# Borda/pyImSegm

Hardware: NVIDIA H100
Metric: megapixels/sec end-to-end SLIC+features+GC (pipe_color2d_slic_features_model_graphcut) (higher is better)
Workload: dtype f64

## Files before the change

include/imsegm_b200.h:

```cpp
#ifndef IMSEGM_B200_H
#define IMSEGM_B200_H

#include <stddef.h>
#include <stdint.h>

#ifdef __cplusplus
extern "C" {
#endif

typedef void* isb_stream_t;

enum isb_status {
    ISB_OK = 0,
    ISB_ERR_ARG = -1,
    ISB_ERR_CUDA = -2,
    ISB_ERR_CAPACITY = -3,
    ISB_ERR_UNSUPPORTED = -4
};

enum isb_dtype { ISB_U8 = 0, ISB_U16 = 1, ISB_F32 = 2, ISB_F64 = 3 };

const char* isb_last_error(void);
int isb_abi_version(void);
long long isb_launch_count(void);
// ... 2 lines not shown
int isb_profile_stage_count(void);
const char* isb_profile_stage_name(int id);
int isb_profile_collect(double* ms_out , long long* count_out );


int isb_slic_prepare(const void* img, int dtype, int H, int W, int C, const double* w_half, int radius, double ratio,
                     int rescale, double* lab_planar, double* minmax_out , isb_stream_t stream);

int isb_image_minmax(const void* img, int dtype, long long n, double* minmax_out , isb_stream_t stream);

size_t isb_slic_kmeans_workspace_bytes(int H, int W, int n_seeds, int step_y, int step_x);

int isb_slic_kmeans(const double* lab_planar, int H, int W, const double* seeds_yx, int n_seeds, int step_y, int step_x,
                    double step, int max_iter, int slic_zero, int32_t* labels, double* centroids, void* ws, size_t ws_bytes,
                    isb_stream_t stream);

typedef struct isb_slic_band {
    int32_t slab_rows, width;
    int32_t image_rows, y_off;
    int32_t own_lo, own_hi;
    int32_t halo;
    int32_t n_seeds, step_y, step_x, slic_zero;
    double step;
    const double* lab_slab;
    size_t plane_stride;
    const double* seeds_yx;
    int32_t* labels_slab;
    void* ws; size_t ws_bytes;
} isb_slic_band_t;
int isb_slic_band_begin(const isb_slic_band_t* band, isb_stream_t stream);
// ... 161 lines not shown
```

pyimsegm_b200/_lib.py:

```python
import ctypes as C
import os

_HERE = os.path.dirname(os.path.abspath(__file__))
LIB_PATH = os.path.join(_HERE, 'libimsegm_b200.so')

_lib = None

ISB_OK, ISB_ERR_ARG, ISB_ERR_CUDA, ISB_ERR_CAPACITY, ISB_ERR_UNSUPPORTED = 0, -1, -2, -3, -4
DTYPE_CODES = {'uint8': 0, 'uint16': 1, 'float32': 2, 'float64': 3}

_vp, _i, _d, _sz, _ll = C.c_void_p, C.c_int, C.c_double, C.c_size_t, C.c_longlong



class SlicBand(C.Structure):
    _fields_ = [('slab_rows', C.c_int32), ('width', C.c_int32), ('image_rows', C.c_int32), ('y_off', C.c_int32),
                ('own_lo', C.c_int32), ('own_hi', C.c_int32), ('halo', C.c_int32),
                ('n_seeds', C.c_int32), ('step_y', C.c_int32), ('step_x', C.c_int32), ('slic_zero', C.c_int32),
                ('step', C.c_double), ('lab_slab', C.c_void_p), ('plane_stride', C.c_size_t), ('seeds_yx', C.c_void_p),
                ('labels_slab', C.c_void_p), ('ws', C.c_void_p), ('ws_bytes', C.c_size_t)]


_bp = C.POINTER(SlicBand)

# ... 6 lines not shown
    'isb_profile_stage_count': (_i, []),
    'isb_profile_stage_name': (C.c_char_p, [_i]),
    'isb_profile_collect': (_i, [C.POINTER(_d), C.POINTER(_ll)]),
    'isb_slic_prepare': (_i, [_vp, _i, _i, _i, _i, C.POINTER(_d), _i, _d, _i, _vp, _vp, _vp]),
    'isb_image_minmax': (_i, [_vp, _i, _ll, _vp, _vp]),
    'isb_slic_band_begin': (_i, [_bp, _vp]),
    'isb_slic_band_assign': (_i, [_bp, _vp]),
    'isb_slic_band_update': (_i, [_bp, _vp, _vp]),
    'isb_slic_band_import': (_i, [_bp, _vp, _vp, _vp]),
    'isb_slic_band_finalize': (_i, [_bp, _vp, _vp]),
    'isb_segment_stats_accumulate': (_i, [_vp, _i, _vp, _i, _i, _i, _i, _vp, _vp, _vp]),
    'isb_segment_stats_deviation': (_i, [_vp, _i, _vp, _i, _i, _i, _vp, _vp, _vp, _vp, _vp]),
    'isb_segment_stats_finish': (_i, [_i, _i, _vp, _vp, _vp, _vp, _i, _i, _vp, _vp, _vp]),
    'isb_slic_kmeans_workspace_bytes': (_sz, [_i, _i, _i, _i, _i]),
    'isb_slic_kmeans': (_i, [_vp, _i, _i, _vp, _i, _i, _i, _d, _i, _i, _vp, _vp, _vp, _sz, _vp]),
    'isb_slic3d_prepare': (_i, [_vp, _i, _i, _i, _i, _vp, _i, _vp, _i, _vp, _i, _d, _vp, _vp, _vp]),
    'isb_slic3d_kmeans_workspace_bytes': (_sz, [_i, _i, _i, _i]),
    'isb_slic3d_kmeans': (_i, [_vp, _i, _i, _i, _vp, _i, _i, _i, _i, _d, C.POINTER(_d), _i, _vp, _vp, _sz, _vp]),
    'isb_connectivity3d_workspace_bytes': (_sz, [_i, _i, _i, _i]),
    'isb_enforce_connectivity3d': (_i, [_vp, _i, _i, _i, _i, _i, _vp, _vp, _vp, _sz, _vp]),
    'isb_connectivity_workspace_bytes': (_sz, [_i, _i]),
    'isb_enforce_connectivity': (_i, [_vp, _i, _i, _i, _i, _vp, _vp, _vp, _sz, _vp]),
    'isb_segment_stats_workspace_bytes': (_sz, [_i]),
    'isb_segment_stats_2d': (_i, [_vp, _i, _vp, _i, _i, _i, _i, _vp, _i, _i, _vp, _vp, _vp, _sz, _vp]),
    'isb_adjacency_workspace_bytes': (_sz, [_i, _i]),
    'isb_adjacency_edges': (_i, [_vp, _i, _i, _i, _vp, _i, _vp, _vp, _sz, _vp]),
    'isb_adjacency_edges_3d': (_i, [_vp, _i, _i, _i, _i, _vp, _i, _vp, _vp, _sz, _vp]),
    'isb_centroids_3d': (_i, [_vp, _i, _i, _i, _i, _vp, _vp, _sz, _vp]),
    'isb_gc_energies_workspace_bytes': (_sz, [_i, _i, _i]),
    'isb_gc_energies': (_i, [_vp, _i, _vp, _i, _vp, _i, _vp, _vp, _i, _i, _d, _vp, _vp, _vp, _vp, _vp, _vp, _vp, _sz, _vp]),
# ... 99 lines not shown
```

pyimsegm_b200/csrc/slic_kmeans.cu:

```cuda
#include "common.cuh"
#include "wgmma.cuh"
#include <float.h>
#include <string.h>

namespace {

constexpr int TILE = 32;
constexpr int ACAP = 128;
constexpr int AROWS = 8;
constexpr int AWARPS = TILE / AROWS;
constexpr int ATHREADS = 32 * AWARPS;


struct __align__(16) Cand {
    double cy, cx, c0, c1, c2;
    int y0, y1, x0, x1;
    int k, pad;
};
static_assert(sizeof(Cand) == 64, "Cand must be 64 bytes");

struct KmState {
    double* cy; double* cx; double* c0; double* c1; double* c2;
    int4* win;
    int4* obb;
    int* bin_start;
    int* bin_fill;
    int* bin_of;
    int* pack_done;
    Cand* packed;
    double* packed_maxdc;
    unsigned long long* maxdc;
    int slico;
    int n, H, W, step_y, step_x, B, nby, nbx;
    double sw;
    int Hg, y_off, own_lo, own_hi, halo;
    size_t pstride;
};

__device__ __forceinline__ int4 make_window(double cy, double cx, int step_y, int step_x, int H, int W)
{
    double lo, hi;
    int4 w;
    lo = __dsub_rn(cy, (double)(2 * step_y)); if (0.0 > lo) lo = 0.0;
    hi = __dadd_rn(__dadd_rn(cy, (double)(2 * step_y)), 1.0); if ((double)H < hi) hi = (double)H;
    w.x = (int)lo; w.y = (int)hi;
    lo = __dsub_rn(cx, (double)(2 * step_x)); if (0.0 > lo) lo = 0.0;
    hi = __dadd_rn(__dadd_rn(cx, (double)(2 * step_x)), 1.0); if ((double)W < hi) hi = (double)W;
    w.z = (int)lo; w.w = (int)hi;
    return w;
}

__global__ void k_seed(KmState s, const double* __restrict__ seeds_yx)
{
    const int k = blockIdx.x * blockDim.x + threadIdx.x;
    if (k >= s.n) return;
    const double cy = seeds_yx[2 * k], cx = seeds_yx[2 * k + 1];
    s.cy[k] = cy; s.cx[k] = cx; s.c0[k] = 0.0; s.c1[k] = 0.0; s.c2[k] = 0.0;
    s.win[k] = make_window(cy, cx, s.step_y, s.step_x, s.Hg, s.W);
    const int by = min(max((int)cy / s.B, 0), s.nby - 1), bx = min(max((int)cx / s.B, 0), s.nbx - 1);
    s.bin_of[k] = by * s.nbx + bx;
    atomicAdd(&s.bin_fill[by * s.nbx + bx], 1);
    s.obb[k] = make_int4(INT_MAX, -1, INT_MAX, -1);
    s.maxdc[k] = (unsigned long long)__double_as_longlong(1.0);
}

__global__ void __launch_bounds__(1024) k_scan_bins(KmState s)
{
    const int nbins = s.nby * s.nbx;
    __shared__ int s_wsum[32];
    __shared__ int s_part_total;
    __shared__ int s_carry;
    if (threadIdx.x == 0) { s_carry = 0; *s.pack_done = 0; }
    __syncthreads();
    const int lane = threadIdx.x & 31, wid = threadIdx.x >> 5, nw = blockDim.x >> 5;
    for (int base = 0; base < nbins; base += blockDim.x) {
        int b = base + threadIdx.x;
        int v = b < nbins ? s.bin_fill[b] : 0;
        int incl = v;
#pragma unroll
        for (int o = 1; o < 32; o <<= 1) { int t = __shfl_up_sync(0xffffffffu, incl, o); if (lane >= o) incl += t; }
        if (lane == 31) s_wsum[wid] = incl;
        __syncthreads();
        if (wid == 0) {
            int t = lane < nw ? s_wsum[lane] : 0, ti = t;
#pragma unroll
            for (int o = 1; o < 32; o <<= 1) { int u = __shfl_up_sync(0xffffffffu, ti, o); if (lane >= o) ti += u; }
            s_wsum[lane] = ti - t;
            if (lane == 31) s_part_total = ti;
        }
        __syncthreads();
        const int carry = s_carry;
        if (b < nbins) { s.bin_start[b] = carry + s_wsum[wid] + incl - v; s.bin_fill[b] = 0; }
        __syncthreads();
        if (threadIdx.x == 0) s_carry = carry + s_part_total;
        __syncthreads();
    }
    if (threadIdx.x == 0) s.bin_start[nbins] = s_carry;
}

__global__ void __launch_bounds__(256) k_pack(KmState s)
{
    const int k = blockIdx.x * blockDim.x + threadIdx.x;
    if (k < s.n) {
        const int bin = s.bin_of[k];
        if (bin >= 0) {
            const int pos = s.bin_start[bin] + atomicAdd(&s.bin_fill[bin], 1);
            const int4 w = s.win[k];
            Cand c;
            c.cy = s.cy[k]; c.cx = s.cx[k]; c.c0 = s.c0[k]; c.c1 = s.c1[k]; c.c2 = s.c2[k];
            c.y0 = w.x; c.y1 = w.y; c.x0 = w.z; c.x1 = w.w; c.k = k; c.pad = 0;
            s.packed[pos] = c;
            if (s.slico) s.packed_maxdc[pos] = __longlong_as_double((long long)s.maxdc[k]);
        }
    }
    __shared__ int s_last;
    __syncthreads();
    if (threadIdx.x == 0) { __threadfence(); s_last = atomicAdd(s.pack_done, 1) == (int)gridDim.x - 1; }
    __syncthreads();
    if (s_last) {
        const int nbins = s.nby * s.nbx;
        for (int b = threadIdx.x; b < nbins; b += blockDim.x) s.bin_fill[b] = 0;
    }
}

__device__ __forceinline__ unsigned long long dbits(double v) { return (unsigned long long)__double_as_longlong(v); }

template <bool SLICO>
__global__ void __launch_bounds__(ATHREADS, 5) k_assign(const __grid_constant__ CUtensorMap lab_map, int use_tma, KmState s,
                                                        const double* __restrict__ lab, int* __restrict__ labels)
{
    __shared__ Cand cand[ACAP];
    __shared__ double s_maxdc[SLICO ? ACAP : 1];
    __shared__ float s_key[ACAP];
    __shared__ float2 s_cf[ACAP];
    __shared__ double s_lb[ACAP];
    __shared__ unsigned char s_order[ACAP];
    __shared__ __align__(128) double s_px[3][TILE][TILE];
    __shared__ __align__(8) unsigned long long s_bar;
    __shared__ int s_ncand, s_done, s_row, s_off, s_total;
    const int tx0 = blockIdx.x * TILE, ty0 = blockIdx.y * TILE;
    const int tx1 = min(tx0 + TILE, s.W);
    const int gy0 = ty0 + s.y_off, gy1 = min(ty0 + TILE, s.H) + s.y_off;
    const int lane = threadIdx.x & 31, warp = threadIdx.x >> 5;
    const size_t HW = s.pstride;
    const int x = tx0 + lane;
    const bool xin = x < s.W;
    const int yb = ty0 + warp * AROWS;

    double best[AROWS];
    int bestk[AROWS];
#pragma unroll
    for (int j = 0; j < AROWS; ++j) { best[j] = DBL_MAX; bestk[j] = -1; }
    if (use_tma) {
        if (threadIdx.x == 0) {
            wgmma::mbar_init(wgmma::smem_u32(&s_bar), 1);
            wgmma::fence_mbar_init();
            wgmma::mbar_arrive_expect_tx(wgmma::smem_u32(&s_bar), 3 * TILE * TILE * 8);
            wgmma::tma_load_3d(wgmma::smem_u32(&s_px[0][0][0]), &lab_map, tx0, ty0, 0, wgmma::smem_u32(&s_bar));
        }
    } else {
        double v[3][AROWS];
#pragma unroll
        for (int j = 0; j < AROWS; ++j) {
            const int y = yb + j;
            if (xin && y < s.H) {
                const size_t p = (size_t)y * s.W + x;
                v[0][j] = lab[p]; v[1][j] = lab[HW + p]; v[2][j] = lab[2 * HW + p];
            } else { v[0][j] = v[1][j] = v[2][j] = 0.0; }
        }
#pragma unroll
        for (int j = 0; j < AROWS; ++j) {
            s_px[0][warp * AROWS + j][lane] = v[0][j]; s_px[1][warp * AROWS + j][lane] = v[1][j]; s_px[2][warp * AROWS + j][lane] = v[2][j];
        }
    }
    const int by0 = max(gy0 - 2 * s.step_y - 2, 0) / s.B, by1 = min(gy1 + 2 * s.step_y + 1, s.Hg - 1) / s.B;
    const int bx0 = max(tx0 - 2 * s.step_x - 2, 0) / s.B, bx1 = min(tx1 + 2 * s.step_x + 1, s.W - 1) / s.B;
    const float tcy = 0.5f * (gy0 + gy1 - 1), tcx = 0.5f * (tx0 + tx1 - 1);
    const int byl = min(by1, s.nby - 1), bxl = min(bx1, s.nbx - 1);
    if (threadIdx.x == 0) { s_row = by0; s_off = 0; s_done = 0; s_ncand = 0; s_total = 0; }
    __syncthreads();
    if (warp == 0) {
        int t = 0;
        for (int row = by0 + lane; row <= byl; row += 32) t += s.bin_start[row * s.nbx + bxl + 1] - s.bin_start[row * s.nbx + bx0];
#pragma unroll
        for (int o = 16; o > 0; o >>= 1) t += __shfl_xor_sync(0xffffffffu, t, o);
        if (lane == 0) s_total = t;
    }
    __syncthreads();
    const bool fast = s_total <= ACAP;

    while (true) {
        if (fast) {
            for (int row = by0 + warp; row <= byl; row += AWARPS) {
                const int beg = s.bin_start[row * s.nbx + bx0], end = s.bin_start[row * s.nbx + bxl + 1];
                for (int i = beg + lane; i < end; i += 32) {
                    const Cand c = s.packed[i];
                    if ((c.y0 < gy1) && (c.y1 > gy0) && (c.x0 < tx1) && (c.x1 > tx0)) {
                        const int pos = atomicAdd(&s_ncand, 1);
                        cand[pos] = c;
                        if (SLICO) s_maxdc[pos] = s.packed_maxdc[i];
                        const float fy = (float)c.cy - tcy, fx = (float)c.cx - tcx;
                        s_key[pos] = fy * fy + fx * fx;
                        s_cf[pos] = make_float2((float)c.cy, (float)c.cx);
                    }
                }
            }
            if (threadIdx.x == 0) s_done = 1;
        } else if (warp == 0) {
            int n = 0;
            int row = s_row, off = s_off;
            while (row <= byl && n < ACAP) {
                int beg = s.bin_start[row * s.nbx + bx0] + off;
                int end = s.bin_start[row * s.nbx + bxl + 1];
                while (beg < end && n < ACAP) {
                    int room = ACAP - n;
                    int i = beg + lane;
                    bool ok = false;
                    Cand c;
                    if (i < end && lane < room) {
                        c = s.packed[i];
                        ok = (c.y0 < gy1) && (c.y1 > gy0) && (c.x0 < tx1) && (c.x1 > tx0);
                    }
                    unsigned m = __ballot_sync(0xffffffffu, ok);
                    if (ok) {
                        int pos = n + __popc(m & ((1u << lane) - 1u));
                        cand[pos] = c;
                        if (SLICO) s_maxdc[pos] = s.packed_maxdc[i];
                        const float fy = (float)c.cy - tcy, fx = (float)c.cx - tcx;
                        s_key[pos] = fy * fy + fx * fx;
                        s_cf[pos] = make_float2((float)c.cy, (float)c.cx);
                    }
                    n += __popc(m);
                    int adv = min(min(32, room), end - beg);
                    beg += adv; off += adv;
                }
                if (beg >= end) { ++row; off = 0; }
            }
            if (lane == 0) { s_ncand = n; s_row = row; s_off = off; s_done = row > byl; }
        }
        __syncthreads();
        const int nc = s_ncand;
        const int done = s_done;
        for (int t = threadIdx.x; t < nc; t += ATHREADS) {
            const float key = s_key[t];
            int rank = 0;
            for (int j = 0; j < nc; ++j) {
                const float kj = s_key[j];
                rank += (kj < key) || (kj == key && j < t);
            }
            s_order[rank] = (unsigned char)t;
            const float r = sqrtf(key) - 23.5f;
            s_lb[rank] = r > 0.f ? (double)(r * r * 0.999f) * s.sw * 0.999 : 0.0;
        }
        __syncthreads();
        if (use_tma) wgmma::mbar_wait(wgmma::smem_u32(&s_bar), 0);
        if (xin) {
            const double xd = (double)x;
            const float xf = (float)x, ymid = (float)(yb + s.y_off) + 0.5f * (AROWS - 1), swf = (float)s.sw * 0.998f;
            unsigned long long worst = dbits(DBL_MAX);
#pragma unroll
            for (int j = 0; j < AROWS; ++j) worst = max(worst, dbits(best[j]));
            float worstf = __double2float_ru(__longlong_as_double((long long)worst));
            for (int ci = 0; ci < nc; ++ci) {
                if (dbits(s_lb[ci]) > worst) break;
                const int c = s_order[ci];
                {
                    const float2 cf = s_cf[c];
                    const float ax = fmaxf(fabsf(cf.y - xf) - 2e-3f, 0.f), ay = fmaxf(fabsf(cf.x - ymid) - (0.5f * (AROWS - 1) + 2e-3f), 0.f);
                    if ((ax * ax + ay * ay) * swf > worstf) continue;
                }
                const int cx0 = cand[c].x0, cx1 = cand[c].x1;
                if (x < cx0 || x >= cx1) continue;
                const int cy0 = cand[c].y0, ck = cand[c].k;
                const unsigned cyn = (unsigned)(cand[c].y1 - cy0);
                const double ccy = cand[c].cy;
                const double tx = __dsub_rn(cand[c].cx, xd);
                const double dx2 = __dmul_rn(tx, tx);
                bool improved = false;
#pragma unroll
                for (int jg = 0; jg < AROWS; jg += 4) {
                    double sp[4];
                    bool need[4];
#pragma unroll
                    for (int q = 0; q < 4; ++q) {
// ... 71 lines not shown
    if (b) asm volatile("bar.arrive %0, %1;" ::"n"(ID + 1), "n"(N) : "memory");
    else asm volatile("bar.arrive %0, %1;" ::"n"(ID), "n"(N) : "memory");
}

template <bool BAND>
__global__ void __launch_bounds__(UTHREADS, UBLOCKS) k_update(KmState s, const double* __restrict__ lab, const int* __restrict__ labels,
                                                              long long* __restrict__ xchg)
{
    __shared__ __align__(16) double buf[2][3][USTRIDE];
    __shared__ int s_cnt[2][USTRIP];
    __shared__ int s_tot[2];
    __shared__ long long s_int[UGATHER][3];
    __shared__ double s_acc[3];
    __shared__ int4 s_box;
    __shared__ int s_skip;
    const int lane = threadIdx.x & 31, wl = threadIdx.x >> 5;
    const int k = s.n - 1 - blockIdx.x;
    if (threadIdx.x == 0) {
        const int4 o = s.obb[k];
        int skip = 0;
        if (BAND) {
            const bool alive = s.bin_of[k] >= 0;
            const int cr = alive ? (int)s.cy[k] : 0;
            if (o.y >= o.x && (!alive || o.x + s.y_off < cr - s.halo || o.y + s.y_off > cr + s.halo))
                atomicAdd((unsigned long long*)&xchg[6 * (size_t)s.n], 1ull);
            s.obb[k] = make_int4(INT_MAX, -1, INT_MAX, -1);
            skip = !alive || cr < s.own_lo || cr >= s.own_hi;
        }
        s_box = o; s_skip = skip;
    }
    __syncthreads();
    if (s_skip) return;
    const int4 o = s_box;
    const int y0 = o.x, y1 = o.y + 1, x0 = o.z, x1 = o.w + 1;
    const int nchunk = (x1 > x0) ? (x1 - x0 + 31) / 32 : 0;
    const int total = (y1 > y0) ? (y1 - y0) * nchunk : 0;
    const int nstrip = (total + USTRIP - 1) / USTRIP;
// ... 72 lines not shown
                const double2* bsrc = reinterpret_cast<const double2*>(buf[b][lane]);
                const int ng = (s_tot[b] + 3) >> 2;
                double2 c01 = bsrc[0], c23 = bsrc[1];
                for (int g = 1; g <= ng; ++g) {
                    const double2 n01 = bsrc[2 * g], n23 = bsrc[2 * g + 1];
                    acc = __dadd_rn(__dadd_rn(__dadd_rn(__dadd_rn(acc, c01.x), c01.y), c23.x), c23.y);
                    c01 = n01; c23 = n23;
                }
            }
            __syncwarp();
            if (i + 2 < nstrip) bar_arrive<UBAR_EMPTY, UTHREADS>(b);
        }
        if (lane < 3) s_acc[lane] = acc;
    }
    __syncthreads();
    if (threadIdx.x != 0) return;
    long long cnt = 0, sy = 0, sx = 0;
#pragma unroll
    for (int w = 0; w < UGATHER; ++w) { cnt += s_int[w][0]; sy += s_int[w][1]; sx += s_int[w][2]; }
    const double a0 = s_acc[0], a1 = s_acc[1], a2 = s_acc[2];
    if (BAND) {
        long long* r = xchg + 6 * (size_t)k;
        if (cnt > 0) {
            const double dn = (double)cnt;
            r[0] = __double_as_longlong(__ddiv_rn((double)sy, dn)); r[1] = __double_as_longlong(__ddiv_rn((double)sx, dn));
            r[2] = __double_as_longlong(__ddiv_rn(a0, dn)); r[3] = __double_as_longlong(__ddiv_rn(a1, dn));
            r[4] = __double_as_longlong(__ddiv_rn(a2, dn));
            r[5] = 1;
        } else r[5] = 2;
        return;
    }
    int4 w = make_int4(0, 0, 0, 0);
    int bin = -1;
    if (cnt > 0) {
        const double dn = (double)cnt;
        const double cy = __ddiv_rn((double)sy, dn), cx = __ddiv_rn((double)sx, dn);
        s.cy[k] = cy; s.cx[k] = cx;
        s.c0[k] = __ddiv_rn(a0, dn); s.c1[k] = __ddiv_rn(a1, dn); s.c2[k] = __ddiv_rn(a2, dn);
        w = make_window(cy, cx, s.step_y, s.step_x, s.Hg, s.W);
        const int by = min(max((int)cy / s.B, 0), s.nby - 1), bx = min(max((int)cx / s.B, 0), s.nbx - 1);
        bin = by * s.nbx + bx;
        atomicAdd(&s.bin_fill[bin], 1);
    }
    s.win[k] = w;
    s.bin_of[k] = bin;
    s.obb[k] = make_int4(INT_MAX, -1, INT_MAX, -1);
}

__global__ void k_import(KmState s, const long long* __restrict__ xchg)
{
    const int k = blockIdx.x * blockDim.x + threadIdx.x;
    if (k >= s.n) return;
    const long long* r = xchg + 6 * (size_t)k;
    const long long state = r[5];
    if (state == 1) {
        const double cy = __longlong_as_double(r[0]), cx = __longlong_as_double(r[1]);
        s.cy[k] = cy; s.cx[k] = cx;
        s.c0[k] = __longlong_as_double(r[2]); s.c1[k] = __longlong_as_double(r[3]); s.c2[k] = __longlong_as_double(r[4]);
        s.win[k] = make_window(cy, cx, s.step_y, s.step_x, s.Hg, s.W);
        const int by = min(max((int)cy / s.B, 0), s.nby - 1), bx = min(max((int)cx / s.B, 0), s.nbx - 1);
        s.bin_of[k] = by * s.nbx + bx;
        atomicAdd(&s.bin_fill[by * s.nbx + bx], 1);
    } else {
        s.win[k] = make_int4(0, 0, 0, 0);
        s.bin_of[k] = -1;
    }
}

__global__ void __launch_bounds__(256) k_slico_max(KmState s, const double* __restrict__ lab, const int* __restrict__ labels)
{
    const size_t HW = s.pstride;
    const size_t first = (size_t)(s.own_lo - s.y_off) * s.W, npx = (size_t)(s.own_hi - s.own_lo) * s.W;
    const size_t q = (size_t)blockIdx.x * blockDim.x + threadIdx.x;
    if (q >= npx) return;
    const size_t p = first + q;
    const int k = labels[p];
    const double d0 = __dsub_rn(lab[p], s.c0[k]), d1 = __dsub_rn(lab[HW + p], s.c1[k]), d2 = __dsub_rn(lab[2 * HW + p], s.c2[k]);
    double dcol = __dmul_rn(d0, d0);
    dcol = __dadd_rn(dcol, __dmul_rn(d1, d1));
    dcol = __dadd_rn(dcol, __dmul_rn(d2, d2));
    if (dcol == dcol) atomicMax(&s.maxdc[k], (unsigned long long)__double_as_longlong(dcol));
}

__global__ void k_export_centroids(KmState s, double* out)
{
    int k = blockIdx.x * blockDim.x + threadIdx.x;
    if (k >= s.n) return;
    out[5 * k] = s.cy[k]; out[5 * k + 1] = s.cx[k];
    out[5 * k + 2] = s.c0[k]; out[5 * k + 3] = s.c1[k]; out[5 * k + 4] = s.c2[k];
}

static size_t carve(KmState& s, void* ws, size_t bytes, int H, int W, int n, int step_y, int step_x)
{
    WsCarver c(ws, bytes);
    s.n = n; s.H = H; s.W = W; s.step_y = step_y; s.step_x = step_x;
    s.Hg = H; s.y_off = 0; s.own_lo = 0; s.own_hi = H; s.halo = 0; s.pstride = (size_t)H * W;
    s.B = 2 * (step_y > step_x ? step_y : step_x);
    if (s.B < 16) s.B = 16;
    s.nby = (H + s.B - 1) / s.B; s.nbx = (W + s.B - 1) / s.B;
    s.cy = c.take<double>(n); s.cx = c.take<double>(n);
    s.c0 = c.take<double>(n); s.c1 = c.take<double>(n); s.c2 = c.take<double>(n);
    s.win = c.take<int4>(n); s.obb = c.take<int4>(n);
    s.bin_start = c.take<int>((size_t)s.nby * s.nbx + 1);
    s.bin_fill = c.take<int>((size_t)s.nby * s.nbx);
    s.bin_of = c.take<int>(n);
    s.pack_done = c.take<int>(1);
    s.packed = c.take<Cand>(n);
    s.maxdc = c.take<unsigned long long>(n);
    s.packed_maxdc = c.take<double>(n);
    return isb_align(c.off);
}

static int rebin(KmState& s, const double* seeds_yx, cudaStream_t st)
{
    if (seeds_yx) {
        ISB_CUDA_CHECK(cudaMemsetAsync(s.bin_fill, 0, sizeof(int) * (size_t)s.nby * s.nbx, st));
        k_seed<<<(s.n + 255) / 256, 256, 0, st>>>(s, seeds_yx);
        ISB_LAUNCH_CHECK();
    }
    k_scan_bins<<<1, 1024, 0, st>>>(s);
    ISB_LAUNCH_CHECK();
    k_pack<<<(s.n + 255) / 256, 256, 0, st>>>(s);
    ISB_LAUNCH_CHECK();
    return ISB_OK;
}

static bool make_lab_map(CUtensorMap& map, const double* lab, int rows, int W, size_t plane_stride)
{
    wgmma::EncodeTiledFn encode = wgmma::encode_tiled_fn();
    if (!encode || (W & 1) || (plane_stride & 1) || ((uintptr_t)lab & 15)) return false;
    const cuuint64_t gdim[3] = { (cuuint64_t)W, (cuuint64_t)rows, 3 };
    const cuuint64_t gstride[2] = { (cuuint64_t)W * sizeof(double), (cuuint64_t)plane_stride * sizeof(double) };
    const cuuint32_t box[3] = { TILE, TILE, 3 };
    const cuuint32_t estr[3] = { 1, 1, 1 };
    return encode(&map, CU_TENSOR_MAP_DATA_TYPE_FLOAT64, 3, (void*)lab, gdim, gstride, box, estr, CU_TENSOR_MAP_INTERLEAVE_NONE,
                  CU_TENSOR_MAP_SWIZZLE_NONE, CU_TENSOR_MAP_L2_PROMOTION_L2_256B, CU_TENSOR_MAP_FLOAT_OOB_FILL_NONE) == CUDA_SUCCESS;
}
// ... 14 lines not shown
}

extern "C" int isb_slic_kmeans(const double* lab_planar, int H, int W, const double* seeds_yx, int n_seeds, int step_y,
                               int step_x, double step, int max_iter, int slic_zero, int32_t* labels, double* centroids,
                               void* ws, size_t ws_bytes, isb_stream_t stream)
{
    ISB_REQUIRE(lab_planar && seeds_yx && labels && ws, "null pointer");
    ISB_REQUIRE(H > 0 && W > 0 && n_seeds > 0 && step_y > 0 && step_x > 0 && step > 0, "bad sizes");
    KmState s;
    size_t need = carve(s, ws, ws_bytes, H, W, n_seeds, step_y, step_x);
    ISB_REQUIRE(need <= ws_bytes, "workspace too small");
    s.sw = 1.0 / (step * step);
    s.slico = slic_zero ? 1 : 0;
    cudaStream_t st = (cudaStream_t)stream;
    ISB_CUDA_CHECK(cudaMemsetAsync(labels, 0, sizeof(int32_t) * (size_t)H * W, st));
    if (int rc = rebin(s, seeds_yx, st)) return rc;
    CUtensorMap lab_map;
    memset(&lab_map, 0, sizeof(lab_map));
    const int use_tma = make_lab_map(lab_map, lab_planar, H, W, s.pstride) ? 1 : 0;
    for (int it = 0; it < max_iter; ++it) {
        {
            ProfScope p(ISB_PROF_ASSIGN, st);
            launch_assign(s, lab_map, use_tma, lab_planar, labels, st);
        }
        ISB_LAUNCH_CHECK();
        { ProfScope p(ISB_PROF_UPDATE, st); k_update<false><<<n_seeds, UTHREADS, 0, st>>>(s, lab_planar, labels, nullptr); }
        ISB_LAUNCH_CHECK();
        if (slic_zero) {
            const size_t npx = (size_t)H * W;
            k_slico_max<<<(unsigned)((npx + 255) / 256), 256, 0, st>>>(s, lab_planar, labels);
            ISB_LAUNCH_CHECK();
        }
        { ProfScope p(ISB_PROF_FINALIZE, st); if (int rc = rebin(s, nullptr, st)) return rc; }
    }
    if (centroids) {
        k_export_centroids<<<(n_seeds + 255) / 256, 256, 0, st>>>(s, centroids);
        ISB_LAUNCH_CHECK();
    }
    return ISB_OK;
}

namespace {

static int band_state(const isb_slic_band_t* b, KmState& s)
{
    ISB_REQUIRE(b && b->lab_slab && b->seeds_yx && b->labels_slab && b->ws, "null pointer");
    ISB_REQUIRE(b->slab_rows > 0 && b->width > 0 && b->image_rows > 0 && b->n_seeds > 0 && b->step_y > 0 && b->step_x > 0 && b->step > 0,
                "bad sizes");
// ... 9 lines not shown
    s.H = b->slab_rows; s.Hg = b->image_rows; s.y_off = b->y_off; s.own_lo = b->own_lo; s.own_hi = b->own_hi; s.halo = b->halo;
    s.pstride = b->plane_stride;
    s.sw = 1.0 / (b->step * b->step);
    s.slico = b->slic_zero ? 1 : 0;
    return ISB_OK;
}

}

extern "C" int isb_slic_band_begin(const isb_slic_band_t* b, isb_stream_t stream)
{
    KmState s;
    if (int rc = band_state(b, s)) return rc;
    cudaStream_t st = (cudaStream_t)stream;
    ISB_CUDA_CHECK(cudaMemsetAsync(b->labels_slab, 0, sizeof(int32_t) * (size_t)b->slab_rows * b->width, st));
    return rebin(s, b->seeds_yx, st);
}

extern "C" int isb_slic_band_assign(const isb_slic_band_t* b, isb_stream_t stream)
{
    KmState s;
    if (int rc = band_state(b, s)) return rc;
    cudaStream_t st = (cudaStream_t)stream;
    CUtensorMap lab_map;
    memset(&lab_map, 0, sizeof(lab_map));
    const int use_tma = make_lab_map(lab_map, b->lab_slab, s.H, s.W, s.pstride) ? 1 : 0;
    ProfScope p(ISB_PROF_ASSIGN, st);
    launch_assign(s, lab_map, use_tma, b->lab_slab, b->labels_slab, st);
    ISB_LAUNCH_CHECK();
    return ISB_OK;
}
// ... 25 lines not shown
        ISB_LAUNCH_CHECK();
        ISB_CUDA_CHECK(cudaMemcpyAsync(maxdc_xchg, s.maxdc, sizeof(uint64_t) * (size_t)s.n, cudaMemcpyDeviceToDevice, st));
    }
    return ISB_OK;
}

extern "C" int isb_slic_band_finalize(const isb_slic_band_t* b, const uint64_t* maxdc_xchg, isb_stream_t stream)
{
    KmState s;
    if (int rc = band_state(b, s)) return rc;
    cudaStream_t st = (cudaStream_t)stream;
    if (s.slico) {
        ISB_REQUIRE(maxdc_xchg, "null pointer");
        ISB_CUDA_CHECK(cudaMemcpyAsync(s.maxdc, maxdc_xchg, sizeof(uint64_t) * (size_t)s.n, cudaMemcpyDeviceToDevice, st));
    }
    ProfScope p(ISB_PROF_FINALIZE, st);
    return rebin(s, nullptr, st);
}
```

Before: 1381.

## Replace seed binning with per-tile candidate lists and add a color-bound prune

Drops the bin scan/pack pipeline (scan_bins and pack kernels run every iteration). The update kernel now appends each centroid straight into per-tile candidate lists via atomics, and the assign kernel reads its own tile's list directly, falling back to a full scan when a tile overflows its capacity. The assign loop also adds a color-space lower bound from per-warp pixel min/max in float with directed rounding, to skip distance evaluations. The cost is tile-list memory, atomic contention, and nondeterministic candidate order, plus a tile-cap knob and a full-scan counter for testing.

```diff
diff --git a/include/imsegm_b200.h b/include/imsegm_b200.h
--- a/include/imsegm_b200.h
+++ b/include/imsegm_b200.h
@@ -40,6 +40,9 @@
 int isb_slic_kmeans(const double* lab_planar, int H, int W, const double* seeds_yx, int n_seeds, int step_y, int step_x,
                     double step, int max_iter, int slic_zero, int32_t* labels, double* centroids, void* ws, size_t ws_bytes,
                     isb_stream_t stream);
+
+int isb_slic_set_tile_cap(int cap);
+long long isb_slic_full_scan_tiles(void);
 
 typedef struct isb_slic_band {
     int32_t slab_rows, width;
diff --git a/pyimsegm_b200/_lib.py b/pyimsegm_b200/_lib.py
--- a/pyimsegm_b200/_lib.py
+++ b/pyimsegm_b200/_lib.py
@@ -44,6 +44,8 @@
     'isb_segment_stats_finish': (_i, [_i, _i, _vp, _vp, _vp, _vp, _i, _i, _vp, _vp, _vp]),
     'isb_slic_kmeans_workspace_bytes': (_sz, [_i, _i, _i, _i, _i]),
     'isb_slic_kmeans': (_i, [_vp, _i, _i, _vp, _i, _i, _i, _d, _i, _i, _vp, _vp, _vp, _sz, _vp]),
+    'isb_slic_set_tile_cap': (_i, [_i]),
+    'isb_slic_full_scan_tiles': (_ll, []),
     'isb_slic3d_prepare': (_i, [_vp, _i, _i, _i, _i, _vp, _i, _vp, _i, _vp, _i, _d, _vp, _vp, _vp]),
     'isb_slic3d_kmeans_workspace_bytes': (_sz, [_i, _i, _i, _i]),
     'isb_slic3d_kmeans': (_i, [_vp, _i, _i, _i, _vp, _i, _i, _i, _i, _d, C.POINTER(_d), _i, _vp, _vp, _sz, _vp]),
diff --git a/pyimsegm_b200/csrc/slic_kmeans.cu b/pyimsegm_b200/csrc/slic_kmeans.cu
--- a/pyimsegm_b200/csrc/slic_kmeans.cu
+++ b/pyimsegm_b200/csrc/slic_kmeans.cu
@@ -23,15 +23,11 @@
     double* cy; double* cx; double* c0; double* c1; double* c2;
     int4* win;
     int4* obb;
-    int* bin_start;
-    int* bin_fill;
-    int* bin_of;
-    int* pack_done;
-    Cand* packed;
-    double* packed_maxdc;
+    int* tile_cnt;
+    Cand* tile_cand;
     unsigned long long* maxdc;
     int slico;
-    int n, H, W, step_y, step_x, B, nby, nbx;
+    int n, H, W, step_y, step_x, ntx, tcap;
     double sw;
     int Hg, y_off, own_lo, own_hi, halo;
     size_t pstride;
@@ -50,115 +46,93 @@
     return w;
 }
 
+__device__ __forceinline__ Cand make_cand(int k, double cy, double cx, double c0, double c1, double c2, int4 w)
+{
+    Cand c;
+    c.cy = cy; c.cx = cx; c.c0 = c0; c.c1 = c1; c.c2 = c2;
+    c.y0 = w.x; c.y1 = w.y; c.x0 = w.z; c.x1 = w.w; c.k = k; c.pad = 0;
+    return c;
+}
+
+__device__ __forceinline__ void append_tiles(const KmState& s, const Cand& c, int t, int nt)
+{
+    const int ya = max(c.y0 - s.y_off, 0), yb = min(c.y1 - s.y_off, s.H);
+    if (ya >= yb || c.x0 >= c.x1) return;
+    const int ty0 = ya / TILE, tx0 = c.x0 / TILE;
+    const int nx = (c.x1 - 1) / TILE - tx0 + 1, nxy = ((yb - 1) / TILE - ty0 + 1) * nx;
+    for (int i = t; i < nxy; i += nt) {
+        const int tile = (ty0 + i / nx) * s.ntx + tx0 + i % nx;
+        const int pos = atomicAdd(&s.tile_cnt[tile], 1);
+        if (pos < s.tcap) s.tile_cand[(size_t)tile * s.tcap + pos] = c;
+    }
+}
+
 __global__ void k_seed(KmState s, const double* __restrict__ seeds_yx)
 {
     const int k = blockIdx.x * blockDim.x + threadIdx.x;
     if (k >= s.n) return;
     const double cy = seeds_yx[2 * k], cx = seeds_yx[2 * k + 1];
     s.cy[k] = cy; s.cx[k] = cx; s.c0[k] = 0.0; s.c1[k] = 0.0; s.c2[k] = 0.0;
-    s.win[k] = make_window(cy, cx, s.step_y, s.step_x, s.Hg, s.W);
-    const int by = min(max((int)cy / s.B, 0), s.nby - 1), bx = min(max((int)cx / s.B, 0), s.nbx - 1);
-    s.bin_of[k] = by * s.nbx + bx;
-    atomicAdd(&s.bin_fill[by * s.nbx + bx], 1);
+    const int4 w = make_window(cy, cx, s.step_y, s.step_x, s.Hg, s.W);
+    s.win[k] = w;
     s.obb[k] = make_int4(INT_MAX, -1, INT_MAX, -1);
     s.maxdc[k] = (unsigned long long)__double_as_longlong(1.0);
-}
-
-__global__ void __launch_bounds__(1024) k_scan_bins(KmState s)
-{
-    const int nbins = s.nby * s.nbx;
-    __shared__ int s_wsum[32];
-    __shared__ int s_part_total;
-    __shared__ int s_carry;
-    if (threadIdx.x == 0) { s_carry = 0; *s.pack_done = 0; }
-    __syncthreads();
-    const int lane = threadIdx.x & 31, wid = threadIdx.x >> 5, nw = blockDim.x >> 5;
-    for (int base = 0; base < nbins; base += blockDim.x) {
-        int b = base + threadIdx.x;
-        int v = b < nbins ? s.bin_fill[b] : 0;
-        int incl = v;
-#pragma unroll
-        for (int o = 1; o < 32; o <<= 1) { int t = __shfl_up_sync(0xffffffffu, incl, o); if (lane >= o) incl += t; }
-        if (lane == 31) s_wsum[wid] = incl;
-        __syncthreads();
-        if (wid == 0) {
-            int t = lane < nw ? s_wsum[lane] : 0, ti = t;
-#pragma unroll
-            for (int o = 1; o < 32; o <<= 1) { int u = __shfl_up_sync(0xffffffffu, ti, o); if (lane >= o) ti += u; }
-            s_wsum[lane] = ti - t;
-            if (lane == 31) s_part_total = ti;
-        }
-        __syncthreads();
-        const int carry = s_carry;
-        if (b < nbins) { s.bin_start[b] = carry + s_wsum[wid] + incl - v; s.bin_fill[b] = 0; }
-        __syncthreads();
-        if (threadIdx.x == 0) s_carry = carry + s_part_total;
-        __syncthreads();
-    }
-    if (threadIdx.x == 0) s.bin_start[nbins] = s_carry;
-}
-
-__global__ void __launch_bounds__(256) k_pack(KmState s)
-{
-    const int k = blockIdx.x * blockDim.x + threadIdx.x;
-    if (k < s.n) {
-        const int bin = s.bin_of[k];
-        if (bin >= 0) {
-            const int pos = s.bin_start[bin] + atomicAdd(&s.bin_fill[bin], 1);
-            const int4 w = s.win[k];
-            Cand c;
-            c.cy = s.cy[k]; c.cx = s.cx[k]; c.c0 = s.c0[k]; c.c1 = s.c1[k]; c.c2 = s.c2[k];
-            c.y0 = w.x; c.y1 = w.y; c.x0 = w.z; c.x1 = w.w; c.k = k; c.pad = 0;
-            s.packed[pos] = c;
-            if (s.slico) s.packed_maxdc[pos] = __longlong_as_double((long long)s.maxdc[k]);
-        }
-    }
-    __shared__ int s_last;
-    __syncthreads();
-    if (threadIdx.x == 0) { __threadfence(); s_last = atomicAdd(s.pack_done, 1) == (int)gridDim.x - 1; }
-    __syncthreads();
-    if (s_last) {
-        const int nbins = s.nby * s.nbx;
-        for (int b = threadIdx.x; b < nbins; b += blockDim.x) s.bin_fill[b] = 0;
-    }
+    append_tiles(s, make_cand(k, cy, cx, 0.0, 0.0, 0.0, w), 0, 1);
 }
 
 __device__ __forceinline__ unsigned long long dbits(double v) { return (unsigned long long)__double_as_longlong(v); }
+
+__device__ unsigned long long d_full_scans;
+
+struct __align__(16) CandF {
+    float cy, cx, inv, pad0;
+    float lo0, lo1, lo2, pad1;
+    float hi0, hi1, hi2, pad2;
+};
 
 template <bool SLICO>
 __global__ void __launch_bounds__(ATHREADS, 5) k_assign(const __grid_constant__ CUtensorMap lab_map, int use_tma, KmState s,
                                                         const double* __restrict__ lab, int* __restrict__ labels)
 {
-    __shared__ Cand cand[ACAP];
+    __shared__ __align__(16) Cand cand[ACAP];
     __shared__ double s_maxdc[SLICO ? ACAP : 1];
     __shared__ float s_key[ACAP];
-    __shared__ float2 s_cf[ACAP];
+    __shared__ CandF s_cf[ACAP];
     __shared__ double s_lb[ACAP];
     __shared__ unsigned char s_order[ACAP];
     __shared__ __align__(128) double s_px[3][TILE][TILE];
     __shared__ __align__(8) unsigned long long s_bar;
-    __shared__ int s_ncand, s_done, s_row, s_off, s_total;
+    __shared__ int s_ncand, s_done;
     const int tx0 = blockIdx.x * TILE, ty0 = blockIdx.y * TILE;
     const int tx1 = min(tx0 + TILE, s.W);
     const int gy0 = ty0 + s.y_off, gy1 = min(ty0 + TILE, s.H) + s.y_off;
+    const int tile = blockIdx.y * s.ntx + blockIdx.x;
     const int lane = threadIdx.x & 31, warp = threadIdx.x >> 5;
     const size_t HW = s.pstride;
     const int x = tx0 + lane;
     const bool xin = x < s.W;
     const int yb = ty0 + warp * AROWS;
+    const uint32_t bar = wgmma::smem_u32(&s_bar);
 
     double best[AROWS];
     int bestk[AROWS];
 #pragma unroll
     for (int j = 0; j < AROWS; ++j) { best[j] = DBL_MAX; bestk[j] = -1; }
-    if (use_tma) {
-        if (threadIdx.x == 0) {
-            wgmma::mbar_init(wgmma::smem_u32(&s_bar), 1);
-            wgmma::fence_mbar_init();
-            wgmma::mbar_arrive_expect_tx(wgmma::smem_u32(&s_bar), 3 * TILE * TILE * 8);
-            wgmma::tma_load_3d(wgmma::smem_u32(&s_px[0][0][0]), &lab_map, tx0, ty0, 0, wgmma::smem_u32(&s_bar));
-        }
-    } else {
+    if (threadIdx.x == 0 && use_tma) {
+        wgmma::mbar_init(bar, 1);
+        wgmma::fence_mbar_init();
+        wgmma::mbar_arrive_expect_tx(bar, 3 * TILE * TILE * 8);
+        wgmma::tma_load_3d(wgmma::smem_u32(&s_px[0][0][0]), &lab_map, tx0, ty0, 0, bar);
+    }
+    const int total = s.tile_cnt[tile];
+    const bool scan_all = total > s.tcap;
+    const bool fast = total <= ACAP && !scan_all;
+    if (fast) {
+        const int4* src = reinterpret_cast<const int4*>(s.tile_cand + (size_t)tile * s.tcap);
+        int4* dst = reinterpret_cast<int4*>(cand);
+        for (int i = threadIdx.x; i < total * (int)(sizeof(Cand) / sizeof(int4)); i += ATHREADS) dst[i] = src[i];
+    }
+    if (!use_tma) {
         double v[3][AROWS];
 #pragma unroll
         for (int j = 0; j < AROWS; ++j) {
@@ -173,74 +147,59 @@
             s_px[0][warp * AROWS + j][lane] = v[0][j]; s_px[1][warp * AROWS + j][lane] = v[1][j]; s_px[2][warp * AROWS + j][lane] = v[2][j];
         }
     }
-    const int by0 = max(gy0 - 2 * s.step_y - 2, 0) / s.B, by1 = min(gy1 + 2 * s.step_y + 1, s.Hg - 1) / s.B;
-    const int bx0 = max(tx0 - 2 * s.step_x - 2, 0) / s.B, bx1 = min(tx1 + 2 * s.step_x + 1, s.W - 1) / s.B;
     const float tcy = 0.5f * (gy0 + gy1 - 1), tcx = 0.5f * (tx0 + tx1 - 1);
-    const int byl = min(by1, s.nby - 1), bxl = min(bx1, s.nbx - 1);
-    if (threadIdx.x == 0) { s_row = by0; s_off = 0; s_done = 0; s_ncand = 0; s_total = 0; }
     __syncthreads();
-    if (warp == 0) {
-        int t = 0;
-        for (int row = by0 + lane; row <= byl; row += 32) t += s.bin_start[row * s.nbx + bxl + 1] - s.bin_start[row * s.nbx + bx0];
-#pragma unroll
-        for (int o = 16; o > 0; o >>= 1) t += __shfl_xor_sync(0xffffffffu, t, o);
-        if (lane == 0) s_total = t;
-    }
-    __syncthreads();
-    const bool fast = s_total <= ACAP;
-
+    if (threadIdx.x == 0) {
+        s.tile_cnt[tile] = 0;
+        if (scan_all) atomicAdd(&d_full_scans, 1ull);
+    }
+
+    int off = 0;
     while (true) {
-        if (fast) {
-            for (int row = by0 + warp; row <= byl; row += AWARPS) {
-                const int beg = s.bin_start[row * s.nbx + bx0], end = s.bin_start[row * s.nbx + bxl + 1];
-                for (int i = beg + lane; i < end; i += 32) {
-                    const Cand c = s.packed[i];
-                    if ((c.y0 < gy1) && (c.y1 > gy0) && (c.x0 < tx1) && (c.x1 > tx0)) {
-                        const int pos = atomicAdd(&s_ncand, 1);
-                        cand[pos] = c;
-                        if (SLICO) s_maxdc[pos] = s.packed_maxdc[i];
-                        const float fy = (float)c.cy - tcy, fx = (float)c.cx - tcx;
-                        s_key[pos] = fy * fy + fx * fx;
-                        s_cf[pos] = make_float2((float)c.cy, (float)c.cx);
+        if (!fast && warp == 0) {
+            const int end = scan_all ? s.n : total;
+            int n = 0;
+            while (off < end && n < ACAP) {
+                const int room = ACAP - n;
+                const int i = off + lane;
+                bool ok = false;
+                Cand c;
+                if (i < end && lane < room) {
+                    if (scan_all) {
+                        const int4 w = s.win[i];
+                        ok = (w.x < gy1) && (w.y > gy0) && (w.z < tx1) && (w.w > tx0);
+                        if (ok) c = make_cand(i, s.cy[i], s.cx[i], s.c0[i], s.c1[i], s.c2[i], w);
+                    } else {
+                        c = s.tile_cand[(size_t)tile * s.tcap + i];
+                        ok = true;
                     }
                 }
-            }
-            if (threadIdx.x == 0) s_done = 1;
-        } else if (warp == 0) {
-            int n = 0;
-            int row = s_row, off = s_off;
-            while (row <= byl && n < ACAP) {
-                int beg = s.bin_start[row * s.nbx + bx0] + off;
-                int end = s.bin_start[row * s.nbx + bxl + 1];
-                while (beg < end && n < ACAP) {
-                    int room = ACAP - n;
-                    int i = beg + lane;
-                    bool ok = false;
-                    Cand c;
-                    if (i < end && lane < room) {
-                        c = s.packed[i];
-                        ok = (c.y0 < gy1) && (c.y1 > gy0) && (c.x0 < tx1) && (c.x1 > tx0);
-                    }
-                    unsigned m = __ballot_sync(0xffffffffu, ok);
-                    if (ok) {
-                        int pos = n + __popc(m & ((1u << lane) - 1u));
-                        cand[pos] = c;
-                        if (SLICO) s_maxdc[pos] = s.packed_maxdc[i];
-                        const float fy = (float)c.cy - tcy, fx = (float)c.cx - tcx;
-                        s_key[pos] = fy * fy + fx * fx;
-                        s_cf[pos] = make_float2((float)c.cy, (float)c.cx);
-                    }
-                    n += __popc(m);
-                    int adv = min(min(32, room), end - beg);
-                    beg += adv; off += adv;
-                }
-                if (beg >= end) { ++row; off = 0; }
-            }
-            if (lane == 0) { s_ncand = n; s_row = row; s_off = off; s_done = row > byl; }
+                const unsigned m = __ballot_sync(0xffffffffu, ok);
+                if (ok) cand[n + __popc(m & ((1u << lane) - 1u))] = c;
+                n += __popc(m);
+                off += min(min(32, room), end - off);
+            }
+            if (lane == 0) { s_ncand = n; s_done = off >= end; }
+        }
+        if (!fast) __syncthreads();
+        const int nc = fast ? total : s_ncand;
+        const int done = fast || s_done;
+        for (int t = threadIdx.x; t < nc; t += ATHREADS) {
+            const Cand& c = cand[t];
+            const float fy = (float)c.cy - tcy, fx = (float)c.cx - tcx;
+            s_key[t] = fy * fy + fx * fx;
+            CandF f;
+            f.cy = (float)c.cy; f.cx = (float)c.cx; f.inv = 1.f; f.pad0 = f.pad1 = f.pad2 = 0.f;
+            f.lo0 = __double2float_rd(c.c0); f.lo1 = __double2float_rd(c.c1); f.lo2 = __double2float_rd(c.c2);
+            f.hi0 = __double2float_ru(c.c0); f.hi1 = __double2float_ru(c.c1); f.hi2 = __double2float_ru(c.c2);
+            if (SLICO) {
+                const double m = __longlong_as_double((long long)s.maxdc[c.k]);
+                s_maxdc[t] = m;
+                f.inv = __frcp_rd(__double2float_ru(m));
+            }
+            s_cf[t] = f;
         }
         __syncthreads();
-        const int nc = s_ncand;
-        const int done = s_done;
         for (int t = threadIdx.x; t < nc; t += ATHREADS) {
             const float key = s_key[t];
             int rank = 0;
@@ -253,7 +212,18 @@
             s_lb[rank] = r > 0.f ? (double)(r * r * 0.999f) * s.sw * 0.999 : 0.0;
         }
         __syncthreads();
-        if (use_tma) wgmma::mbar_wait(wgmma::smem_u32(&s_bar), 0);
+        if (use_tma) wgmma::mbar_wait(bar, 0);
+        float plo0 = INFINITY, plo1 = INFINITY, plo2 = INFINITY, phi0 = -INFINITY, phi1 = -INFINITY, phi2 = -INFINITY;
+#pragma unroll
+        for (int j = 0; j < AROWS; ++j) {
+            if (yb + j < s.H) {
+                const int ry = warp * AROWS + j;
+                const double v0 = s_px[0][ry][lane], v1 = s_px[1][ry][lane], v2 = s_px[2][ry][lane];
+                plo0 = fminf(plo0, __double2float_rd(v0)); phi0 = fmaxf(phi0, __double2float_ru(v0));
+                plo1 = fminf(plo1, __double2float_rd(v1)); phi1 = fmaxf(phi1, __double2float_ru(v1));
+                plo2 = fminf(plo2, __double2float_rd(v2)); phi2 = fmaxf(phi2, __double2float_ru(v2));
+            }
+        }
         if (xin) {
             const double xd = (double)x;
             const float xf = (float)x, ymid = (float)(yb + s.y_off) + 0.5f * (AROWS - 1), swf = (float)s.sw * 0.998f;
@@ -265,9 +235,16 @@
                 if (dbits(s_lb[ci]) > worst) break;
                 const int c = s_order[ci];
                 {
-                    const float2 cf = s_cf[c];
-                    const float ax = fmaxf(fabsf(cf.y - xf) - 2e-3f, 0.f), ay = fmaxf(fabsf(cf.x - ymid) - (0.5f * (AROWS - 1) + 2e-3f), 0.f);
-                    if ((ax * ax + ay * ay) * swf > worstf) continue;
+                    const CandF f = s_cf[c];
+                    const float ax = fmaxf(fabsf(f.cx - xf) - 2e-3f, 0.f), ay = fmaxf(fabsf(f.cy - ymid) - (0.5f * (AROWS - 1) + 2e-3f), 0.f);
+                    const float lbs = (ax * ax + ay * ay) * swf;
+                    if (lbs > worstf) continue;
+                    const float g0 = fmaxf(fmaxf(__fsub_rd(plo0, f.hi0), __fsub_rd(f.lo0, phi0)), 0.f);
+                    const float g1 = fmaxf(fmaxf(__fsub_rd(plo1, f.hi1), __fsub_rd(f.lo1, phi1)), 0.f);
+                    const float g2 = fmaxf(fmaxf(__fsub_rd(plo2, f.hi2), __fsub_rd(f.lo2, phi2)), 0.f);
+                    float lbc = __fadd_rd(__fadd_rd(__fmul_rd(g0, g0), __fmul_rd(g1, g1)), __fmul_rd(g2, g2));
+                    if (SLICO) lbc = __fmul_rd(lbc, f.inv);
+                    if (__fmaf_rd(lbc, 0.998f, lbs) > worstf) continue;
                 }
                 const int cx0 = cand[c].x0, cx1 = cand[c].x1;
                 if (x < cx0 || x >= cx1) continue;
@@ -369,13 +346,15 @@
     __shared__ double s_acc[3];
     __shared__ int4 s_box;
     __shared__ int s_skip;
+    __shared__ Cand s_rec;
     const int lane = threadIdx.x & 31, wl = threadIdx.x >> 5;
     const int k = s.n - 1 - blockIdx.x;
     if (threadIdx.x == 0) {
         const int4 o = s.obb[k];
         int skip = 0;
         if (BAND) {
-            const bool alive = s.bin_of[k] >= 0;
+            const int4 w = s.win[k];
+            const bool alive = w.y > w.x;
             const int cr = alive ? (int)s.cy[k] : 0;
             if (o.y >= o.x && (!alive || o.x + s.y_off < cr - s.halo || o.y + s.y_off > cr + s.halo))
                 atomicAdd((unsigned long long*)&xchg[6 * (size_t)s.n], 1ull);
@@ -478,37 +457,38 @@
         if (lane < 3) s_acc[lane] = acc;
     }
     __syncthreads();
-    if (threadIdx.x != 0) return;
-    long long cnt = 0, sy = 0, sx = 0;
-#pragma unroll
-    for (int w = 0; w < UGATHER; ++w) { cnt += s_int[w][0]; sy += s_int[w][1]; sx += s_int[w][2]; }
-    const double a0 = s_acc[0], a1 = s_acc[1], a2 = s_acc[2];
-    if (BAND) {
-        long long* r = xchg + 6 * (size_t)k;
-        if (cnt > 0) {
-            const double dn = (double)cnt;
-            r[0] = __double_as_longlong(__ddiv_rn((double)sy, dn)); r[1] = __double_as_longlong(__ddiv_rn((double)sx, dn));
-            r[2] = __double_as_longlong(__ddiv_rn(a0, dn)); r[3] = __double_as_longlong(__ddiv_rn(a1, dn));
-            r[4] = __double_as_longlong(__ddiv_rn(a2, dn));
-            r[5] = 1;
-        } else r[5] = 2;
-        return;
-    }
-    int4 w = make_int4(0, 0, 0, 0);
-    int bin = -1;
-    if (cnt > 0) {
-        const double dn = (double)cnt;
-        const double cy = __ddiv_rn((double)sy, dn), cx = __ddiv_rn((double)sx, dn);
-        s.cy[k] = cy; s.cx[k] = cx;
-        s.c0[k] = __ddiv_rn(a0, dn); s.c1[k] = __ddiv_rn(a1, dn); s.c2[k] = __ddiv_rn(a2, dn);
-        w = make_window(cy, cx, s.step_y, s.step_x, s.Hg, s.W);
-        const int by = min(max((int)cy / s.B, 0), s.nby - 1), bx = min(max((int)cx / s.B, 0), s.nbx - 1);
-        bin = by * s.nbx + bx;
-        atomicAdd(&s.bin_fill[bin], 1);
-    }
-    s.win[k] = w;
-    s.bin_of[k] = bin;
-    s.obb[k] = make_int4(INT_MAX, -1, INT_MAX, -1);
+    if (wl != 0) return;
+    if (lane == 0) {
+        long long cnt = 0, sy = 0, sx = 0;
+#pragma unroll
+        for (int w = 0; w < UGATHER; ++w) { cnt += s_int[w][0]; sy += s_int[w][1]; sx += s_int[w][2]; }
+        const double a0 = s_acc[0], a1 = s_acc[1], a2 = s_acc[2];
+        if (BAND) {
+            long long* r = xchg + 6 * (size_t)k;
+            if (cnt > 0) {
+                const double dn = (double)cnt;
+                r[0] = __double_as_longlong(__ddiv_rn((double)sy, dn)); r[1] = __double_as_longlong(__ddiv_rn((double)sx, dn));
+                r[2] = __double_as_longlong(__ddiv_rn(a0, dn)); r[3] = __double_as_longlong(__ddiv_rn(a1, dn));
+                r[4] = __double_as_longlong(__ddiv_rn(a2, dn));
+                r[5] = 1;
+            } else r[5] = 2;
+        } else {
+            int4 w = make_int4(0, 0, 0, 0);
+            if (cnt > 0) {
+                const double dn = (double)cnt;
+                const double cy = __ddiv_rn((double)sy, dn), cx = __ddiv_rn((double)sx, dn);
+                const double c0 = __ddiv_rn(a0, dn), c1 = __ddiv_rn(a1, dn), c2 = __ddiv_rn(a2, dn);
+                s.cy[k] = cy; s.cx[k] = cx; s.c0[k] = c0; s.c1[k] = c1; s.c2[k] = c2;
+                w = make_window(cy, cx, s.step_y, s.step_x, s.Hg, s.W);
+                s_rec = make_cand(k, cy, cx, c0, c1, c2, w);
+            } else s_rec.y0 = s_rec.y1 = 0;
+            s.win[k] = w;
+            s.obb[k] = make_int4(INT_MAX, -1, INT_MAX, -1);
+        }
+    }
+    if (BAND) return;
+    __syncwarp();
+    append_tiles(s, s_rec, lane, 32);
 }
 
 __global__ void k_import(KmState s, const long long* __restrict__ xchg)
@@ -521,13 +501,11 @@
         const double cy = __longlong_as_double(r[0]), cx = __longlong_as_double(r[1]);
         s.cy[k] = cy; s.cx[k] = cx;
         s.c0[k] = __longlong_as_double(r[2]); s.c1[k] = __longlong_as_double(r[3]); s.c2[k] = __longlong_as_double(r[4]);
-        s.win[k] = make_window(cy, cx, s.step_y, s.step_x, s.Hg, s.W);
-        const int by = min(max((int)cy / s.B, 0), s.nby - 1), bx = min(max((int)cx / s.B, 0), s.nbx - 1);
-        s.bin_of[k] = by * s.nbx + bx;
-        atomicAdd(&s.bin_fill[by * s.nbx + bx], 1);
+        const int4 w = make_window(cy, cx, s.step_y, s.step_x, s.Hg, s.W);
+        s.win[k] = w;
+        append_tiles(s, make_cand(k, cy, cx, __longlong_as_double(r[2]), __longlong_as_double(r[3]), __longlong_as_double(r[4]), w), 0, 1);
     } else {
         s.win[k] = make_int4(0, 0, 0, 0);
-        s.bin_of[k] = -1;
     }
 }
 
@@ -554,37 +532,30 @@
     out[5 * k + 2] = s.c0[k]; out[5 * k + 3] = s.c1[k]; out[5 * k + 4] = s.c2[k];
 }
 
+static int g_tile_cap = 0;
+
 static size_t carve(KmState& s, void* ws, size_t bytes, int H, int W, int n, int step_y, int step_x)
 {
     WsCarver c(ws, bytes);
     s.n = n; s.H = H; s.W = W; s.step_y = step_y; s.step_x = step_x;
     s.Hg = H; s.y_off = 0; s.own_lo = 0; s.own_hi = H; s.halo = 0; s.pstride = (size_t)H * W;
-    s.B = 2 * (step_y > step_x ? step_y : step_x);
-    if (s.B < 16) s.B = 16;
-    s.nby = (H + s.B - 1) / s.B; s.nbx = (W + s.B - 1) / s.B;
     s.cy = c.take<double>(n); s.cx = c.take<double>(n);
     s.c0 = c.take<double>(n); s.c1 = c.take<double>(n); s.c2 = c.take<double>(n);
     s.win = c.take<int4>(n); s.obb = c.take<int4>(n);
-    s.bin_start = c.take<int>((size_t)s.nby * s.nbx + 1);
-    s.bin_fill = c.take<int>((size_t)s.nby * s.nbx);
-    s.bin_of = c.take<int>(n);
-    s.pack_done = c.take<int>(1);
-    s.packed = c.take<Cand>(n);
     s.maxdc = c.take<unsigned long long>(n);
-    s.packed_maxdc = c.take<double>(n);
+    s.ntx = (W + TILE - 1) / TILE;
+    s.tcap = ((TILE + 4 * step_y + 2) / step_y + 2) * ((TILE + 4 * step_x + 2) / step_x + 2);
+    if (g_tile_cap > 0 && g_tile_cap < s.tcap) s.tcap = g_tile_cap;
+    const size_t tiles = (size_t)((H + TILE - 1) / TILE) * s.ntx;
+    s.tile_cnt = c.take<int>(tiles);
+    s.tile_cand = c.take<Cand>(tiles * s.tcap);
     return isb_align(c.off);
 }
 
-static int rebin(KmState& s, const double* seeds_yx, cudaStream_t st)
-{
-    if (seeds_yx) {
-        ISB_CUDA_CHECK(cudaMemsetAsync(s.bin_fill, 0, sizeof(int) * (size_t)s.nby * s.nbx, st));
-        k_seed<<<(s.n + 255) / 256, 256, 0, st>>>(s, seeds_yx);
-        ISB_LAUNCH_CHECK();
-    }
-    k_scan_bins<<<1, 1024, 0, st>>>(s);
-    ISB_LAUNCH_CHECK();
-    k_pack<<<(s.n + 255) / 256, 256, 0, st>>>(s);
+static int seed(KmState& s, const double* seeds_yx, cudaStream_t st)
+{
+    ISB_CUDA_CHECK(cudaMemsetAsync(s.tile_cnt, 0, sizeof(int) * (size_t)((s.Hg + TILE - 1) / TILE) * s.ntx, st));
+    k_seed<<<(s.n + 255) / 256, 256, 0, st>>>(s, seeds_yx);
     ISB_LAUNCH_CHECK();
     return ISB_OK;
 }
@@ -629,7 +600,7 @@
     s.slico = slic_zero ? 1 : 0;
     cudaStream_t st = (cudaStream_t)stream;
     ISB_CUDA_CHECK(cudaMemsetAsync(labels, 0, sizeof(int32_t) * (size_t)H * W, st));
-    if (int rc = rebin(s, seeds_yx, st)) return rc;
+    if (int rc = seed(s, seeds_yx, st)) return rc;
     CUtensorMap lab_map;
     memset(&lab_map, 0, sizeof(lab_map));
     const int use_tma = make_lab_map(lab_map, lab_planar, H, W, s.pstride) ? 1 : 0;
@@ -646,7 +617,6 @@
             k_slico_max<<<(unsigned)((npx + 255) / 256), 256, 0, st>>>(s, lab_planar, labels);
             ISB_LAUNCH_CHECK();
         }
-        { ProfScope p(ISB_PROF_FINALIZE, st); if (int rc = rebin(s, nullptr, st)) return rc; }
     }
     if (centroids) {
         k_export_centroids<<<(n_seeds + 255) / 256, 256, 0, st>>>(s, centroids);
@@ -686,7 +656,7 @@
     if (int rc = band_state(b, s)) return rc;
     cudaStream_t st = (cudaStream_t)stream;
     ISB_CUDA_CHECK(cudaMemsetAsync(b->labels_slab, 0, sizeof(int32_t) * (size_t)b->slab_rows * b->width, st));
-    return rebin(s, b->seeds_yx, st);
+    return seed(s, b->seeds_yx, st);
 }
 
 extern "C" int isb_slic_band_assign(const isb_slic_band_t* b, isb_stream_t stream)
@@ -742,6 +712,20 @@
         ISB_REQUIRE(maxdc_xchg, "null pointer");
         ISB_CUDA_CHECK(cudaMemcpyAsync(s.maxdc, maxdc_xchg, sizeof(uint64_t) * (size_t)s.n, cudaMemcpyDeviceToDevice, st));
     }
-    ProfScope p(ISB_PROF_FINALIZE, st);
-    return rebin(s, nullptr, st);
-}
+    return ISB_OK;
+}
+
+extern "C" int isb_slic_set_tile_cap(int cap)
+{
+    ISB_REQUIRE(cap >= 0, "bad tile cap");
+    const int prev = g_tile_cap;
+    g_tile_cap = cap;
+    return prev;
+}
+
+extern "C" long long isb_slic_full_scan_tiles(void)
+{
+    unsigned long long v = 0;
+    ISB_CUDA_CHECK(cudaMemcpyFromSymbol(&v, d_full_scans, sizeof(v)));
+    return (long long)v;
+}
```

New measurement: 1429 (median of 6 runs). 3.5% higher.
